# KyanChen/RSPrompter

Measured on NVIDIA H100. Metric: images/sec, higher is better.
Workload: dtype bf16

## Files before the change

rsprompter_b200/csrc/attention.cu:

```cuda
#include <cstdlib>

#include "attention.h"
#include "sm90.cuh"

namespace rsp {

constexpr float LOG2E = 1.4426950408889634f;

__device__ __forceinline__ float fast_exp2(float x) {
  float y;
  asm("ex2.approx.ftz.f32 %0, %1;" : "=f"(y) : "f"(x));
  return y;
}
__device__ __forceinline__ uint32_t pack_f16x2(float lo, float hi) {
  __half2 v = __floats2half2_rn(lo, hi);
  return *reinterpret_cast<uint32_t*>(&v);
}
__device__ __forceinline__ uint32_t bf16x2_to_f16x2(uint32_t w) {
  return pack_f16x2(__uint_as_float(w << 16), __uint_as_float(w & 0xffff0000u));
}

template <int HD, int S>
struct AttCfg {
  static constexpr int T = S * S;
  static constexpr int BM = 128;
  static constexpr int BN = 64;
  static constexpr int NQT = (T + BM - 1) / BM;
  static constexpr int NKT = (T + BN - 1) / BN;
  static constexpr int NREL = 2 * S - 1;
  static constexpr int NTAB = NREL <= 32 ? 32 : (NREL <= 64 ? 64 : 128);
  static constexpr int TAIL = HD - 64;
  static constexpr int STAGES = 4;
  static constexpr int SP = S + 4;
  __host__ __device__ static constexpr int tile_bytes(int rows) { return rows * (128 + 2 * TAIL); }
  static constexpr int STAGE_BYTES = 2 * tile_bytes(BN);
  static constexpr int smem_bytes(int qbuf) {
    return qbuf * tile_bytes(BM) + STAGES * STAGE_BYTES + 2 * tile_bytes(NTAB) + 2 * BM * SP * 4 + 8 * 64 + 1024;
  }
  static constexpr int QBUF = smem_bytes(2) <= 227 * 1024 ? 2 : 1;
  static constexpr int Q_OFF = 0;
  static constexpr int KV_OFF = Q_OFF + QBUF * tile_bytes(BM);
  static constexpr int TAB_OFF = KV_OFF + STAGES * STAGE_BYTES;
  static constexpr int BIAS_OFF = TAB_OFF + 2 * tile_bytes(NTAB);
  static constexpr int BAR_OFF = BIAS_OFF + 2 * BM * SP * 4;
  static constexpr int SMEM_BYTES = smem_bytes(QBUF);
  static constexpr int REG_PRODUCER = 40, REG_CONSUMER = 232;
  static_assert(HD == 64 || HD == 80, "head dim");
  static_assert(NREL <= 128, "table rows");
  static_assert(SMEM_BYTES <= 227 * 1024, "shared memory");
};

struct AttDev {
  __nv_bfloat16* out;
  const int* out_row_map;
  int H;
  int D;
  int n_items;
  float scale2;
};

template <int N, int TAIL>
__device__ __forceinline__ void qk_wgmma(float (&acc)[N / 2], uint32_t qa, uint32_t qtail, uint32_t b, int b_rows) {
  acc_fence(acc);
  wgmma_fence();
#pragma unroll
  for (int k = 0; k < 4; ++k)
    Wgmma<N>::template ss<0>(acc, make_gdesc(qa + 32 * k, 16, 1024), make_gdesc(b + 32 * k, 16, 1024), k);
  if constexpr (TAIL > 0)
    Wgmma<N>::template ss<0>(acc, make_gdesc_sw32(qtail, 16, 256), make_gdesc_sw32(b + b_rows * 128, 16, 256), 1);
  wgmma_commit();
  wgmma_wait<0>();
  acc_fence(acc);
}

template <int TAIL>
__device__ __forceinline__ void load_tile(uint32_t dst, int rows, const CUtensorMap* m, const CUtensorMap* mt,
                                          uint32_t bar, int col, int row, int seq) {
  tma_load_3d(dst, m, bar, col, row, seq);
  if constexpr (TAIL > 0) tma_load_3d(dst + rows * 128, mt, bar, col + 64, row, seq);
}

template <int HD, int S>
__global__ void __launch_bounds__(384, 1)
vit_attention_kernel(const __grid_constant__ CUtensorMap tm_q, const __grid_constant__ CUtensorMap tm_q_t,
                     const __grid_constant__ CUtensorMap tm_kv, const __grid_constant__ CUtensorMap tm_kv_t,
                     const __grid_constant__ CUtensorMap tm_rh, const __grid_constant__ CUtensorMap tm_rh_t,
                     const __grid_constant__ CUtensorMap tm_rw, const __grid_constant__ CUtensorMap tm_rw_t,
                     const AttDev p) {
  using C = AttCfg<HD, S>;
  constexpr int T = C::T, BM = C::BM, BN = C::BN, NKT = C::NKT, SP = C::SP, STAGES = C::STAGES, TAIL = C::TAIL;
  constexpr int QBUF = C::QBUF;
  constexpr uint32_t TILE_KV = C::tile_bytes(BN), TILE_TAB = C::tile_bytes(C::NTAB);
  extern __shared__ __align__(1024) uint8_t smem_raw[];
  uint8_t* smem = smem_raw + ((1024u - (smem_u32(smem_raw) & 1023u)) & 1023u);
  const uint32_t sbase = smem_u32(smem);
  float* relh = reinterpret_cast<float*>(smem + C::BIAS_OFF);
  float* relw = relh + BM * SP;
  uint64_t* bar_tab = reinterpret_cast<uint64_t*>(smem + C::BAR_OFF);
  uint64_t* bar_q = bar_tab + 1;
  uint64_t* bar_qe = bar_q + QBUF;
  uint64_t* bar_k = bar_qe + QBUF;
  uint64_t* bar_v = bar_k + STAGES;
  uint64_t* bar_vc = bar_v + STAGES;
  uint64_t* bar_e = bar_vc + STAGES;

  const int warp = threadIdx.x >> 5, lane = threadIdx.x & 31;
  auto decode = [&](int item, int& q0, int& head, int& seq) {
    q0 = (item % C::NQT) * BM;
    item /= C::NQT;
    head = item % p.H;
    seq = item / p.H;
  };

  if (threadIdx.x == 0) {
    tma_prefetch_desc(&tm_q);
    tma_prefetch_desc(&tm_kv);
    mbar_init(smem_u32(bar_tab), 1);
    for (int b = 0; b < QBUF; ++b) {
      mbar_init(smem_u32(&bar_q[b]), 1);
      mbar_init(smem_u32(&bar_qe[b]), 8);
    }
    for (int s = 0; s < STAGES; ++s) {
      mbar_init(smem_u32(&bar_k[s]), 1);
      mbar_init(smem_u32(&bar_v[s]), 1);
      mbar_init(smem_u32(&bar_vc[s]), 3);
      mbar_init(smem_u32(&bar_e[s]), 8);
    }
    fence_barrier_init();
  }
  __syncthreads();

  if (warp < 4) {
    setmaxnreg_dec<C::REG_PRODUCER>();
    if (warp == 0) {
      if (lane == 0) {
        const uint32_t bq = smem_u32(bar_tab);
        mbar_expect_tx(bq, 2 * TILE_TAB);
        tma_load_2d(sbase + C::TAB_OFF, &tm_rh, bq, 0, 0);
        tma_load_2d(sbase + C::TAB_OFF + TILE_TAB, &tm_rw, bq, 0, 0);
        if constexpr (TAIL > 0) {
          tma_load_2d(sbase + C::TAB_OFF + C::NTAB * 128, &tm_rh_t, bq, 64, 0);
          tma_load_2d(sbase + C::TAB_OFF + TILE_TAB + C::NTAB * 128, &tm_rw_t, bq, 64, 0);
        }
        int g = 0;
#pragma unroll 1
        for (int item = blockIdx.x, it = 0; item < p.n_items; item += gridDim.x, ++it) {
          int q0, head, seq;
          decode(item, q0, head, seq);
          const int colq = head * HD, colk = p.D + colq, colv = 2 * p.D + colq;
          const int qb = it % QBUF;
          mbar_wait(smem_u32(&bar_qe[qb]), ((it / QBUF) & 1) ^ 1);
          mbar_expect_tx(smem_u32(&bar_q[qb]), C::tile_bytes(BM));
          load_tile<TAIL>(sbase + C::Q_OFF + qb * C::tile_bytes(BM), BM, &tm_q, &tm_q_t, smem_u32(&bar_q[qb]),
                          colq, q0, seq);
#pragma unroll 1
          for (int j = 0; j < NKT; ++j, ++g) {
            const int s = g % STAGES;
            mbar_wait(smem_u32(&bar_e[s]), ((g / STAGES) & 1) ^ 1);
            const uint32_t kb = sbase + C::KV_OFF + s * C::STAGE_BYTES;
            mbar_expect_tx(smem_u32(&bar_k[s]), TILE_KV);
            load_tile<TAIL>(kb, BN, &tm_kv, &tm_kv_t, smem_u32(&bar_k[s]), colk, j * BN, seq);
            mbar_expect_tx(smem_u32(&bar_v[s]), TILE_KV);
            load_tile<TAIL>(kb + TILE_KV, BN, &tm_kv, &tm_kv_t, smem_u32(&bar_v[s]), colv, j * BN, seq);
          }
        }
      }
    } else {
      const int t = threadIdx.x - 32;
      const int n_tiles = ((p.n_items - static_cast<int>(blockIdx.x) + gridDim.x - 1) / gridDim.x) * NKT;
#pragma unroll 1
      for (int g = 0; g < n_tiles; ++g) {
        const int s = g % STAGES;
        mbar_wait(smem_u32(&bar_v[s]), (g / STAGES) & 1);
        uint4* v = reinterpret_cast<uint4*>(smem + C::KV_OFF + s * C::STAGE_BYTES + TILE_KV);
#pragma unroll 2
        for (int i = t; i < static_cast<int>(TILE_KV / 16); i += 96) {
          uint4 w = v[i];
          w.x = bf16x2_to_f16x2(w.x);
          w.y = bf16x2_to_f16x2(w.y);
          w.z = bf16x2_to_f16x2(w.z);
          w.w = bf16x2_to_f16x2(w.w);
          v[i] = w;
        }
        fence_proxy_async_smem();
        __syncwarp();
        if (lane == 0) mbar_arrive(smem_u32(&bar_vc[s]));
      }
    }
    return;
  }

  setmaxnreg_inc<C::REG_CONSUMER>();
  const int wg = (warp >> 2) - 1;
  const int r0 = wg * 64 + (warp & 3) * 16 + (lane >> 2);
  const int cq = 2 * (lane & 3);
  constexpr bool REG_W = BN % S == 0;
  constexpr int CPS = REG_W ? S / 8 : 1;
  mbar_wait(smem_u32(bar_tab), 0);
  int g = 0;
#pragma unroll 1
  for (int item = blockIdx.x, it = 0; item < p.n_items; item += gridDim.x, ++it) {
    int q0, head, seq;
    decode(item, q0, head, seq);
    const int qb = it % QBUF;
    const uint32_t qbase = sbase + C::Q_OFF + qb * C::tile_bytes(BM);
    const uint32_t qa = qbase + wg * 64 * 128;
    const uint32_t qtail = qbase + BM * 128 + wg * 64 * 32;

    mbar_wait(smem_u32(&bar_q[qb]), (it / QBUF) & 1);
    named_bar_sync(1 + wg, 128);
#pragma unroll 1
    for (int tab = 0; tab < 2; ++tab) {
      float acc[C::NTAB / 2];
      qk_wgmma<C::NTAB, TAIL>(acc, qa, qtail, sbase + C::TAB_OFF + tab * TILE_TAB, C::NTAB);
      float* dst = tab ? relw : relh;
#pragma unroll
      for (int x = 0; x < C::NTAB / 2; ++x) {
        const int r = r0 + 8 * ((x >> 1) & 1);
        const int tq = q0 + r;
        const int qc = tab ? tq % S : tq / S;
        const int t = 8 * (x >> 2) + cq + (x & 1);
        const int k = qc + S - 1 - t;
        if (t < C::NREL && k >= 0 && k < S) dst[r * SP + k] = acc[x] * LOG2E;
      }
    }
    named_bar_sync(1 + wg, 128);

    float rw[2][2 * CPS];
    if constexpr (REG_W) {
#pragma unroll
      for (int i = 0; i < 2; ++i)
#pragma unroll
        for (int m = 0; m < 2 * CPS; ++m) rw[i][m] = relw[(r0 + 8 * i) * SP + 8 * (m >> 1) + cq + (m & 1)];
    }

    float om[32], ot[8];
#pragma unroll
    for (int y = 0; y < 32; ++y) om[y] = 0.f;
#pragma unroll
    for (int y = 0; y < 8; ++y) ot[y] = 0.f;
    float m_run[2] = {-INFINITY, -INFINITY}, l_run[2] = {0.f, 0.f};
    const float scale2 = p.scale2;

#pragma unroll(REG_W ? 1 : NKT)
    for (int j = 0; j < NKT; ++j, ++g) {
      const int s = g % STAGES;
      const uint32_t ph = (g / STAGES) & 1;
      const uint32_t kb = sbase + C::KV_OFF + s * C::STAGE_BYTES, vb = kb + TILE_KV;
      mbar_wait(smem_u32(&bar_k[s]), ph);
      float sc[BN / 2];
      qk_wgmma<BN, TAIL>(sc, qa, qtail, kb, BN);
      if (j == NKT - 1) {
        __syncwarp();
        if (lane == 0) mbar_arrive(smem_u32(&bar_qe[qb]));
      }

      float mx[2] = {-INFINITY, -INFINITY};
      if constexpr (REG_W) {
        constexpr int NB = BN / S;
        float bh[2][NB];
#pragma unroll
        for (int i = 0; i < 2; ++i)
#pragma unroll
          for (int b = 0; b < NB; ++b) bh[i][b] = relh[(r0 + 8 * i) * SP + j * NB + b];
#pragma unroll
        for (int x = 0; x < BN / 2; ++x) {
          const int i = (x >> 1) & 1;
          const float t = fmaf(sc[x], scale2, bh[i][(x >> 2) / CPS] + rw[i][((x >> 2) % CPS) * 2 + (x & 1)]);
          sc[x] = t;
          mx[i] = fmaxf(mx[i], t);
        }
      } else {
#pragma unroll
        for (int x = 0; x < BN / 2; ++x) {
          const int i = (x >> 1) & 1;
          const int key = j * BN + 8 * (x >> 2) + cq + (x & 1);
          float t = -INFINITY;
          if (T % BN == 0 || key < T) {
            const int kh = key / S, kw = key - kh * S;
            const int r = r0 + 8 * i;
            t = fmaf(sc[x], scale2, relh[r * SP + kh] + relw[r * SP + kw]);
          }
          sc[x] = t;
          mx[i] = fmaxf(mx[i], t);
        }
      }
      float alpha[2];
#pragma unroll
      for (int i = 0; i < 2; ++i) {
        mx[i] = fmaxf(mx[i], __shfl_xor_sync(0xffffffffu, mx[i], 1));
        mx[i] = fmaxf(mx[i], __shfl_xor_sync(0xffffffffu, mx[i], 2));
        const float m_new = fmaxf(m_run[i], mx[i]);
        alpha[i] = fast_exp2(m_run[i] - m_new);
        m_run[i] = m_new;
        l_run[i] *= alpha[i];
      }
#pragma unroll
      for (int y = 0; y < 32; ++y) om[y] *= alpha[(y >> 1) & 1];
#pragma unroll
      for (int y = 0; y < 8; ++y) ot[y] *= alpha[(y >> 1) & 1];
      uint32_t pa[BN / 16][4];
#pragma unroll
      for (int kk = 0; kk < BN / 16; ++kk) {
#pragma unroll
        for (int h = 0; h < 4; ++h) {
          const int x = 8 * kk + 2 * h, i = h & 1;
          const float p0 = fast_exp2(sc[x] - m_run[i]), p1 = fast_exp2(sc[x + 1] - m_run[i]);
          l_run[i] += p0 + p1;
          pa[kk][h] = pack_f16x2(p0, p1);
        }
      }
      mbar_wait(smem_u32(&bar_vc[s]), ph);
      acc_fence(om);
      acc_fence(ot);
      wgmma_fence();
#pragma unroll
      for (int kk = 0; kk < BN / 16; ++kk) {
        WgmmaRsF16<64>::rs(om, pa[kk], make_gdesc(vb + kk * 2048, BN * 128, 1024));
        if constexpr (TAIL > 0) WgmmaRsF16<16>::rs(ot, pa[kk], make_gdesc_sw32(vb + BN * 128 + kk * 512, 256, 256));
      }
      wgmma_commit();
      wgmma_wait<0>();
      acc_fence(om);
      acc_fence(ot);
      __syncwarp();
      if (lane == 0) mbar_arrive(smem_u32(&bar_e[s]));
    }

#pragma unroll
    for (int i = 0; i < 2; ++i) {
      float l = l_run[i];
      l += __shfl_xor_sync(0xffffffffu, l, 1);
      l += __shfl_xor_sync(0xffffffffu, l, 2);
      const float inv = 1.0f / l;
      const int tq = q0 + r0 + 8 * i;
      if (tq >= T) continue;
      int dst = seq * T + tq;
      if (p.out_row_map) dst = __ldg(p.out_row_map + dst);
      if (dst < 0) continue;
      __nv_bfloat16* orow = p.out + static_cast<size_t>(dst) * p.D + head * HD + cq;
#pragma unroll
      for (int nb = 0; nb < 8; ++nb)
        *reinterpret_cast<uint32_t*>(orow + nb * 8) = pack_bf16x2(om[4 * nb + 2 * i] * inv, om[4 * nb + 2 * i + 1] * inv);
      if constexpr (TAIL > 0) {
#pragma unroll
        for (int nb = 0; nb < 2; ++nb)
          *reinterpret_cast<uint32_t*>(orow + 64 + nb * 8) =
              pack_bf16x2(ot[4 * nb + 2 * i] * inv, ot[4 * nb + 2 * i + 1] * inv);
      }
    }
  }
}

template <int HD, int S>
static int launch_att(const AttentionArgs& a, cudaStream_t stream) {
  using C = AttCfg<HD, S>;
  RSP_CHECK_ARG((reinterpret_cast<uintptr_t>(a.qkv) & 15) == 0 && (reinterpret_cast<uintptr_t>(a.rel_h) & 15) == 0 &&
                (reinterpret_cast<uintptr_t>(a.rel_w) & 15) == 0 && (reinterpret_cast<uintptr_t>(a.out) & 3) == 0,
                "attention: qkv / tables must be 16-byte aligned");
  AttDev p;
  p.out = static_cast<__nv_bfloat16*>(a.out);
  p.out_row_map = a.out_row_map;
  p.H = a.H; p.D = a.H * HD;
  p.scale2 = (1.0f / sqrtf(static_cast<float>(HD))) * LOG2E;
  const uint64_t ld = 3ull * p.D;
  const uint64_t qdims[3] = {ld, static_cast<uint64_t>(C::T), static_cast<uint64_t>(a.n_seq)};
  const uint64_t qstr[2] = {ld * 2, ld * 2 * C::T};
  const uint64_t tdims[2] = {static_cast<uint64_t>(HD), static_cast<uint64_t>(C::NREL)};
  const uint64_t tstr[1] = {static_cast<uint64_t>(HD) * 2};
  const uint32_t qbox[3] = {64, C::BM, 1}, qbox_t[3] = {16, C::BM, 1};
  const uint32_t kvbox[3] = {64, C::BN, 1}, kvbox_t[3] = {16, C::BN, 1};
  const uint32_t tbox[2] = {64, static_cast<uint32_t>(C::NTAB)}, tbox_t[2] = {16, static_cast<uint32_t>(C::NTAB)};
  CUtensorMap tq, tkv, th, tw, tq_t, tkv_t, th_t, tw_t;
  RSP_TRY(make_tmap_swizzled(&tq, a.qkv, 3, qdims, qstr, qbox, 0, 128));
  RSP_TRY(make_tmap_swizzled(&tkv, a.qkv, 3, qdims, qstr, kvbox, 0, 128));
  RSP_TRY(make_tmap_swizzled(&th, a.rel_h, 2, tdims, tstr, tbox, 0, 128));
  RSP_TRY(make_tmap_swizzled(&tw, a.rel_w, 2, tdims, tstr, tbox, 0, 128));
  if (C::TAIL > 0) {
    RSP_TRY(make_tmap_swizzled(&tq_t, a.qkv, 3, qdims, qstr, qbox_t, 0, 32));
    RSP_TRY(make_tmap_swizzled(&tkv_t, a.qkv, 3, qdims, qstr, kvbox_t, 0, 32));
    RSP_TRY(make_tmap_swizzled(&th_t, a.rel_h, 2, tdims, tstr, tbox_t, 0, 32));
    RSP_TRY(make_tmap_swizzled(&tw_t, a.rel_w, 2, tdims, tstr, tbox_t, 0, 32));
  } else {
    tq_t = tq; tkv_t = tkv; th_t = th; tw_t = tw;
  }
  auto kern = vit_attention_kernel<HD, S>;
  static bool attr_set_dev[kMaxDevices] = {};
  bool& attr_set = attr_set_dev[current_device()];
  if (!attr_set) {
    RSP_CHECK_CUDA(cudaFuncSetAttribute(kern, cudaFuncAttributeMaxDynamicSharedMemorySize, C::SMEM_BYTES));
    attr_set = true;
  }
  const long long items = static_cast<long long>(a.n_seq) * a.H * C::NQT;
  RSP_CHECK_ARG(items > 0 && items < (1ll << 31), "attention: %lld query tiles", items);
  p.n_items = static_cast<int>(items);
  const int grid = static_cast<int>(items < num_sms() ? items : num_sms());
  kern<<<grid, 384, C::SMEM_BYTES, stream>>>(tq, tq_t, tkv, tkv_t, th, th_t, tw, tw_t, p);
  RSP_CHECK_LAUNCH();
  return RSP_OK;
}

int vit_attention(const AttentionArgs& a, cudaStream_t stream) {
  RSP_CHECK_ARG(a.qkv && a.rel_h && a.rel_w && a.out, "attention: null pointer");
  RSP_CHECK_ARG(a.T == a.S * a.S, "attention: T=%d is not S^2 (S=%d)", a.T, a.S);
  RSP_CHECK_ARG(a.n_seq > 0 && a.H > 0, "attention: bad n_seq/H");
  if (a.S != 14 && a.S != 32 && a.S != 64)
    return vit_attention_simt(a, stream);
  if (a.hd == 64) {
    if (a.S == 64) return launch_att<64, 64>(a, stream);
    if (a.S == 32) return launch_att<64, 32>(a, stream);
    return launch_att<64, 14>(a, stream);
  }
  if (a.hd == 80) {
    if (a.S == 64) return launch_att<80, 64>(a, stream);
    if (a.S == 32) return launch_att<80, 32>(a, stream);
    return launch_att<80, 14>(a, stream);
  }
  set_last_error("attention: head dim %d unsupported (64, 80)", a.hd);
  return RSP_ERR_UNSUPPORTED;
}

__global__ void vit_attention_simt_kernel(const __nv_bfloat16* __restrict__ qkv,
                                          const __nv_bfloat16* __restrict__ rel_h,
                                          const __nv_bfloat16* __restrict__ rel_w,
                                          __nv_bfloat16* __restrict__ out, int T, int S, int H,
                                          int hd, float scale, const int* __restrict__ out_row_map) {
  const int D = H * hd;
  const int tq = blockIdx.x * blockDim.x + threadIdx.x;
  const int head = blockIdx.y;
  const int seq = blockIdx.z;
  if (tq >= T) return;
  const int qh = tq / S, qw = tq % S;
  const __nv_bfloat16* qp = qkv + (static_cast<size_t>(seq) * T + tq) * 3 * D + head * hd;
  float q[128];
  for (int d = 0; d < hd; ++d) q[d] = __bfloat162float(qp[d]);
  float rh[128], rw[128];
  for (int k = 0; k < S; ++k) {
    float ah = 0.f, aw = 0.f;
    const __nv_bfloat16* th = rel_h + static_cast<size_t>(qh - k + S - 1) * hd;
    const __nv_bfloat16* tw = rel_w + static_cast<size_t>(qw - k + S - 1) * hd;
    for (int d = 0; d < hd; ++d) {
      ah += q[d] * __bfloat162float(th[d]);
      aw += q[d] * __bfloat162float(tw[d]);
    }
    rh[k] = ah; rw[k] = aw;
  }
  float m = -INFINITY, l = 0.f;
  float o[128];
  for (int d = 0; d < hd; ++d) o[d] = 0.f;
  for (int k = 0; k < T; ++k) {
    const __nv_bfloat16* kp = qkv + (static_cast<size_t>(seq) * T + k) * 3 * D + D + head * hd;
    const __nv_bfloat16* vp = kp + D;
    float s = 0.f;
    for (int d = 0; d < hd; ++d) s += q[d] * __bfloat162float(kp[d]);
    s = s * scale + rh[k / S] + rw[k % S];
    const float mn = fmaxf(m, s);
    const float a = expf(m - mn), pe = expf(s - mn);
    l = l * a + pe;
    for (int d = 0; d < hd; ++d) o[d] = o[d] * a + pe * __bfloat162float(vp[d]);
    m = mn;
  }
  int dst = seq * T + tq;
  if (out_row_map) dst = out_row_map[dst];
  if (dst < 0) return;
  __nv_bfloat16* op = out + static_cast<size_t>(dst) * D + head * hd;
  for (int d = 0; d < hd; ++d) op[d] = __float2bfloat16_rn(o[d] / l);
}

int vit_attention_simt(const AttentionArgs& a, cudaStream_t stream) {
  RSP_CHECK_ARG(a.qkv && a.rel_h && a.rel_w && a.out, "attention_simt: null pointer");
  RSP_CHECK_ARG(a.T == a.S * a.S && a.S <= 128 && a.hd <= 128, "attention_simt: bad T/S/hd");
  dim3 block(64);
  dim3 grid((a.T + 63) / 64, a.H, a.n_seq);
  vit_attention_simt_kernel<<<grid, block, 0, stream>>>(
      static_cast<const __nv_bfloat16*>(a.qkv), static_cast<const __nv_bfloat16*>(a.rel_h),
      static_cast<const __nv_bfloat16*>(a.rel_w), static_cast<__nv_bfloat16*>(a.out), a.T, a.S, a.H,
      a.hd, 1.0f / sqrtf(static_cast<float>(a.hd)), a.out_row_map);
  RSP_CHECK_LAUNCH();
  return RSP_OK;
}
// ... 3 lines not shown
```

rsprompter_b200/csrc/sm90.cuh:

```cuda
#pragma once
#include <cuda.h>
#include <cuda_bf16.h>
#include <cuda_runtime.h>
#include <stdint.h>

namespace rsp {

__device__ __forceinline__ uint32_t smem_u32(const void* p) {
  return static_cast<uint32_t>(__cvta_generic_to_shared(p));
}

__device__ __forceinline__ uint32_t elect_one() {
  uint32_t pred = 0;
  asm volatile(
      "{\n"
      ".reg .b32 rx;\n"
      ".reg .pred px;\n"
      "elect.sync rx|px, 0xffffffff;\n"
      "selp.u32 %0, 1, 0, px;\n"
      "}\n"
      : "=r"(pred));
  return pred;
}

// ... 22 lines not shown
      "selp.u32 %0, 1, 0, p;\n"
      "}\n"
      : "=r"(ok)
      : "r"(bar), "r"(parity)
      : "memory");
  return ok;
}
__device__ __forceinline__ void mbar_wait(uint32_t bar, uint32_t parity) {
  if (mbar_try_wait(bar, parity)) return;
  long long t0 = clock64();
  uint32_t spins = 0;
  while (!mbar_try_wait(bar, parity)) {
    if ((++spins & 0x3ff) == 0 && clock64() - t0 > (1ll << 31)) __trap();
  }
}

__device__ __forceinline__ void tma_prefetch_desc(const CUtensorMap* m) {
  asm volatile("prefetch.tensormap [%0];" ::"l"(m) : "memory");
}
__device__ __forceinline__ void tma_load_2d(uint32_t dst, const CUtensorMap* m, uint32_t bar,
                                            int c0, int c1) {
  asm volatile(
      "cp.async.bulk.tensor.2d.shared::cluster.global.mbarrier::complete_tx::bytes"
      " [%0], [%1, {%3, %4}], [%2];" ::"r"(dst),
      "l"(m), "r"(bar), "r"(c0), "r"(c1)
      : "memory");
}
__device__ __forceinline__ void tma_load_3d(uint32_t dst, const CUtensorMap* m, uint32_t bar,
                                            int c0, int c1, int c2) {
  asm volatile(
      "cp.async.bulk.tensor.3d.shared::cluster.global.mbarrier::complete_tx::bytes"
      " [%0], [%1, {%3, %4, %5}], [%2];" ::"r"(dst),
      "l"(m), "r"(bar), "r"(c0), "r"(c1), "r"(c2)
      : "memory");
}
__device__ __forceinline__ void tma_load_4d(uint32_t dst, const CUtensorMap* m, uint32_t bar,
                                            int c0, int c1, int c2, int c3) {
  asm volatile(
      "cp.async.bulk.tensor.4d.shared::cluster.global.mbarrier::complete_tx::bytes"
      " [%0], [%1, {%3, %4, %5, %6}], [%2];" ::"r"(dst),
      "l"(m), "r"(bar), "r"(c0), "r"(c1), "r"(c2), "r"(c3)
      : "memory");
}

__device__ __forceinline__ void tma_store_2d(const CUtensorMap* m, uint32_t src, int c0, int c1) {
  asm volatile("cp.async.bulk.tensor.2d.global.shared::cta.bulk_group [%0, {%2, %3}], [%1];" ::"l"(m), "r"(src),
               "r"(c0), "r"(c1)
               : "memory");
}
__device__ __forceinline__ void bulk_commit() { asm volatile("cp.async.bulk.commit_group;" ::: "memory"); }
__device__ __forceinline__ void bulk_wait_read0() { asm volatile("cp.async.bulk.wait_group.read 0;" ::: "memory"); }
__device__ __forceinline__ void bulk_wait0() { asm volatile("cp.async.bulk.wait_group 0;" ::: "memory"); }

__device__ __forceinline__ uint64_t make_gdesc(uint32_t saddr, uint32_t lbo_bytes, uint32_t sbo_bytes) {
  uint64_t d = 0;
  d |= static_cast<uint64_t>((saddr & 0x3ffff) >> 4);
  d |= static_cast<uint64_t>((lbo_bytes >> 4) & 0x3fff) << 16;
  d |= static_cast<uint64_t>((sbo_bytes >> 4) & 0x3fff) << 32;
  d |= 1ull << 62;
  return d;
}

__device__ __forceinline__ uint64_t make_gdesc_sw32(uint32_t saddr, uint32_t lbo_bytes, uint32_t sbo_bytes) {
  uint64_t d = 0;
  d |= static_cast<uint64_t>((saddr & 0x3ffff) >> 4);
  d |= static_cast<uint64_t>((lbo_bytes >> 4) & 0x3fff) << 16;
  d |= static_cast<uint64_t>((sbo_bytes >> 4) & 0x3fff) << 32;
  d |= 3ull << 62;
  return d;
}

__device__ __forceinline__ void wgmma_fence() { asm volatile("wgmma.fence.sync.aligned;" ::: "memory"); }
__device__ __forceinline__ void wgmma_commit() { asm volatile("wgmma.commit_group.sync.aligned;" ::: "memory"); }
template <int N>
__device__ __forceinline__ void wgmma_wait() { asm volatile("wgmma.wait_group.sync.aligned %0;" ::"n"(N) : "memory"); }
template <int R>
__device__ __forceinline__ void acc_fence(float (&d)[R]) {
#pragma unroll
  for (int i = 0; i < R; ++i) asm volatile("" : "+f"(d[i])::"memory");
}

template <int N>
struct Wgmma;
template <> struct Wgmma<32> {
  template <int TB>
  __device__ __forceinline__ static void ss(float (&d)[16], uint64_t a, uint64_t b, uint32_t acc) {
    asm volatile(
        "{\n.reg .pred p;\n"
        "setp.ne.b32 p, %18, 0;\n"
        "wgmma.mma_async.sync.aligned.m64n32k16.f32.bf16.bf16 "
        "{" 
        "%0, %1, %2, %3, %4, %5, %6, %7, %8, %9, %10, %11, %12, %13, %14, %15"
        "}, %16, %17, p, 1, 1, 0, %19;\n}\n"
        : "+f"(d[0]), "+f"(d[1]), "+f"(d[2]), "+f"(d[3]), "+f"(d[4]), "+f"(d[5]), "+f"(d[6]), "+f"(d[7]),
          "+f"(d[8]), "+f"(d[9]), "+f"(d[10]), "+f"(d[11]), "+f"(d[12]), "+f"(d[13]), "+f"(d[14]), "+f"(d[15])
        : "l"(a), "l"(b), "r"(acc), "n"(TB));
  }
};
template <> struct Wgmma<64> {
  template <int TB>
  __device__ __forceinline__ static void ss(float (&d)[32], uint64_t a, uint64_t b, uint32_t acc) {
    asm volatile(
        "{\n.reg .pred p;\n"
        "setp.ne.b32 p, %34, 0;\n"
        "wgmma.mma_async.sync.aligned.m64n64k16.f32.bf16.bf16 "
        "{" 
        "%0, %1, %2, %3, %4, %5, %6, %7, %8, %9, %10, %11, %12, %13, %14, %15, "
        "%16, %17, %18, %19, %20, %21, %22, %23, %24, %25, %26, %27, %28, %29, %30, %31"
        "}, %32, %33, p, 1, 1, 0, %35;\n}\n"
        : "+f"(d[0]), "+f"(d[1]), "+f"(d[2]), "+f"(d[3]), "+f"(d[4]), "+f"(d[5]), "+f"(d[6]), "+f"(d[7]),
          "+f"(d[8]), "+f"(d[9]), "+f"(d[10]), "+f"(d[11]), "+f"(d[12]), "+f"(d[13]), "+f"(d[14]), "+f"(d[15]),
          "+f"(d[16]), "+f"(d[17]), "+f"(d[18]), "+f"(d[19]), "+f"(d[20]), "+f"(d[21]), "+f"(d[22]), "+f"(d[23]),
          "+f"(d[24]), "+f"(d[25]), "+f"(d[26]), "+f"(d[27]), "+f"(d[28]), "+f"(d[29]), "+f"(d[30]), "+f"(d[31])
        : "l"(a), "l"(b), "r"(acc), "n"(TB));
  }
};
template <> struct Wgmma<128> {
  template <int TB>
  __device__ __forceinline__ static void ss(float (&d)[64], uint64_t a, uint64_t b, uint32_t acc) {
    asm volatile(
        "{\n.reg .pred p;\n"
        "setp.ne.b32 p, %66, 0;\n"
        "wgmma.mma_async.sync.aligned.m64n128k16.f32.bf16.bf16 "
        "{" 
        "%0, %1, %2, %3, %4, %5, %6, %7, %8, %9, %10, %11, %12, %13, %14, %15, "
        "%16, %17, %18, %19, %20, %21, %22, %23, %24, %25, %26, %27, %28, %29, %30, %31, "
        "%32, %33, %34, %35, %36, %37, %38, %39, %40, %41, %42, %43, %44, %45, %46, %47, "
        "%48, %49, %50, %51, %52, %53, %54, %55, %56, %57, %58, %59, %60, %61, %62, %63"
        "}, %64, %65, p, 1, 1, 0, %67;\n}\n"
        : "+f"(d[0]), "+f"(d[1]), "+f"(d[2]), "+f"(d[3]), "+f"(d[4]), "+f"(d[5]), "+f"(d[6]), "+f"(d[7]),
          "+f"(d[8]), "+f"(d[9]), "+f"(d[10]), "+f"(d[11]), "+f"(d[12]), "+f"(d[13]), "+f"(d[14]), "+f"(d[15]),
          "+f"(d[16]), "+f"(d[17]), "+f"(d[18]), "+f"(d[19]), "+f"(d[20]), "+f"(d[21]), "+f"(d[22]), "+f"(d[23]),
          "+f"(d[24]), "+f"(d[25]), "+f"(d[26]), "+f"(d[27]), "+f"(d[28]), "+f"(d[29]), "+f"(d[30]), "+f"(d[31]),
          "+f"(d[32]), "+f"(d[33]), "+f"(d[34]), "+f"(d[35]), "+f"(d[36]), "+f"(d[37]), "+f"(d[38]), "+f"(d[39]),
          "+f"(d[40]), "+f"(d[41]), "+f"(d[42]), "+f"(d[43]), "+f"(d[44]), "+f"(d[45]), "+f"(d[46]), "+f"(d[47]),
          "+f"(d[48]), "+f"(d[49]), "+f"(d[50]), "+f"(d[51]), "+f"(d[52]), "+f"(d[53]), "+f"(d[54]), "+f"(d[55]),
          "+f"(d[56]), "+f"(d[57]), "+f"(d[58]), "+f"(d[59]), "+f"(d[60]), "+f"(d[61]), "+f"(d[62]), "+f"(d[63])
        : "l"(a), "l"(b), "r"(acc), "n"(TB));
  }
};
template <> struct Wgmma<256> {
  template <int TB>
  __device__ __forceinline__ static void ss(float (&d)[128], uint64_t a, uint64_t b, uint32_t acc) {
    asm volatile(
        "{\n.reg .pred p;\n"
        "setp.ne.b32 p, %130, 0;\n"
        "wgmma.mma_async.sync.aligned.m64n256k16.f32.bf16.bf16 "
        "{" 
        "%0, %1, %2, %3, %4, %5, %6, %7, %8, %9, %10, %11, %12, %13, %14, %15, "
        "%16, %17, %18, %19, %20, %21, %22, %23, %24, %25, %26, %27, %28, %29, %30, %31, "
        "%32, %33, %34, %35, %36, %37, %38, %39, %40, %41, %42, %43, %44, %45, %46, %47, "
        "%48, %49, %50, %51, %52, %53, %54, %55, %56, %57, %58, %59, %60, %61, %62, %63, "
        "%64, %65, %66, %67, %68, %69, %70, %71, %72, %73, %74, %75, %76, %77, %78, %79, "
        "%80, %81, %82, %83, %84, %85, %86, %87, %88, %89, %90, %91, %92, %93, %94, %95, "
        "%96, %97, %98, %99, %100, %101, %102, %103, %104, %105, %106, %107, %108, %109, %110, %111, "
        "%112, %113, %114, %115, %116, %117, %118, %119, %120, %121, %122, %123, %124, %125, %126, %127"
        "}, %128, %129, p, 1, 1, 0, %131;\n}\n"
        : "+f"(d[0]), "+f"(d[1]), "+f"(d[2]), "+f"(d[3]), "+f"(d[4]), "+f"(d[5]), "+f"(d[6]), "+f"(d[7]),
          "+f"(d[8]), "+f"(d[9]), "+f"(d[10]), "+f"(d[11]), "+f"(d[12]), "+f"(d[13]), "+f"(d[14]), "+f"(d[15]),
          "+f"(d[16]), "+f"(d[17]), "+f"(d[18]), "+f"(d[19]), "+f"(d[20]), "+f"(d[21]), "+f"(d[22]), "+f"(d[23]),
          "+f"(d[24]), "+f"(d[25]), "+f"(d[26]), "+f"(d[27]), "+f"(d[28]), "+f"(d[29]), "+f"(d[30]), "+f"(d[31]),
          "+f"(d[32]), "+f"(d[33]), "+f"(d[34]), "+f"(d[35]), "+f"(d[36]), "+f"(d[37]), "+f"(d[38]), "+f"(d[39]),
          "+f"(d[40]), "+f"(d[41]), "+f"(d[42]), "+f"(d[43]), "+f"(d[44]), "+f"(d[45]), "+f"(d[46]), "+f"(d[47]),
          "+f"(d[48]), "+f"(d[49]), "+f"(d[50]), "+f"(d[51]), "+f"(d[52]), "+f"(d[53]), "+f"(d[54]), "+f"(d[55]),
          "+f"(d[56]), "+f"(d[57]), "+f"(d[58]), "+f"(d[59]), "+f"(d[60]), "+f"(d[61]), "+f"(d[62]), "+f"(d[63]),
          "+f"(d[64]), "+f"(d[65]), "+f"(d[66]), "+f"(d[67]), "+f"(d[68]), "+f"(d[69]), "+f"(d[70]), "+f"(d[71]),
// ... 179 lines not shown
```

Measured before the change: 61.08.

## Add window-attention path with whole-sequence items, trimmed tail tiles, and pipelined wgmma

For the S=14 window case (T=196, not a multiple of BN), each work item now covers a whole sequence and head. All Q rows are loaded once and the K/V tiles stay resident across the query tiles. The last K/V tile is loaded with narrower TMA boxes (8 and 16 rows) and computed with a new m64n8 wgmma, so less padding is loaded and multiplied. The per-tile loop is software-pipelined so the next QK wgmma and the previous PV wgmma overlap the softmax, and relative-position biases are held in registers. In exchange it uses more shared memory for Q, more registers, and gives fewer, larger work items, which can hurt load balance.

After: 62.36, median of 6. +2.1%, better.

```diff
diff --git a/rsprompter_b200/csrc/attention.cu b/rsprompter_b200/csrc/attention.cu
--- a/rsprompter_b200/csrc/attention.cu
+++ b/rsprompter_b200/csrc/attention.cu
@@ -1,4 +1,5 @@
 #include <cstdlib>
+#include <type_traits>
 
 #include "attention.h"
 #include "sm90.cuh"
@@ -27,6 +28,10 @@
   static constexpr int BN = 64;
   static constexpr int NQT = (T + BM - 1) / BM;
   static constexpr int NKT = (T + BN - 1) / BN;
+  static constexpr bool WIN = T % BN != 0;
+  static constexpr int QROWS = WIN ? NQT * BM : BM;
+  static constexpr int KT = WIN ? (T - (NKT - 1) * BN + 7) / 8 * 8 : BN;
+  static constexpr int VT = WIN ? (T - (NKT - 1) * BN + 15) / 16 * 16 : BN;
   static constexpr int NREL = 2 * S - 1;
   static constexpr int NTAB = NREL <= 32 ? 32 : (NREL <= 64 ? 64 : 128);
   static constexpr int TAIL = HD - 64;
@@ -35,11 +40,11 @@
   __host__ __device__ static constexpr int tile_bytes(int rows) { return rows * (128 + 2 * TAIL); }
   static constexpr int STAGE_BYTES = 2 * tile_bytes(BN);
   static constexpr int smem_bytes(int qbuf) {
-    return qbuf * tile_bytes(BM) + STAGES * STAGE_BYTES + 2 * tile_bytes(NTAB) + 2 * BM * SP * 4 + 8 * 64 + 1024;
+    return qbuf * tile_bytes(QROWS) + STAGES * STAGE_BYTES + 2 * tile_bytes(NTAB) + 2 * BM * SP * 4 + 8 * 64 + 1024;
   }
   static constexpr int QBUF = smem_bytes(2) <= 227 * 1024 ? 2 : 1;
   static constexpr int Q_OFF = 0;
-  static constexpr int KV_OFF = Q_OFF + QBUF * tile_bytes(BM);
+  static constexpr int KV_OFF = Q_OFF + QBUF * tile_bytes(QROWS);
   static constexpr int TAB_OFF = KV_OFF + STAGES * STAGE_BYTES;
   static constexpr int BIAS_OFF = TAB_OFF + 2 * tile_bytes(NTAB);
   static constexpr int BAR_OFF = BIAS_OFF + 2 * BM * SP * 4;
@@ -48,6 +53,7 @@
   static_assert(HD == 64 || HD == 80, "head dim");
   static_assert(NREL <= 128, "table rows");
   static_assert(SMEM_BYTES <= 227 * 1024, "shared memory");
+  static_assert(!WIN || (S == 14 && STAGES == NKT && KT == 8 && VT == 16 && QBUF == 2), "window tiling");
 };
 
 struct AttDev {
@@ -86,11 +92,13 @@
                      const __grid_constant__ CUtensorMap tm_kv, const __grid_constant__ CUtensorMap tm_kv_t,
                      const __grid_constant__ CUtensorMap tm_rh, const __grid_constant__ CUtensorMap tm_rh_t,
                      const __grid_constant__ CUtensorMap tm_rw, const __grid_constant__ CUtensorMap tm_rw_t,
-                     const AttDev p) {
+                     const AttDev p,
+                     const __grid_constant__ CUtensorMap tm_kt, const __grid_constant__ CUtensorMap tm_kt_t,
+                     const __grid_constant__ CUtensorMap tm_vt, const __grid_constant__ CUtensorMap tm_vt_t) {
   using C = AttCfg<HD, S>;
   constexpr int T = C::T, BM = C::BM, BN = C::BN, NKT = C::NKT, SP = C::SP, STAGES = C::STAGES, TAIL = C::TAIL;
   constexpr int QBUF = C::QBUF;
-  constexpr uint32_t TILE_KV = C::tile_bytes(BN), TILE_TAB = C::tile_bytes(C::NTAB);
+  constexpr uint32_t TILE_KV = C::tile_bytes(BN), TILE_TAB = C::tile_bytes(C::NTAB), TILE_Q = C::tile_bytes(C::QROWS);
   extern __shared__ __align__(1024) uint8_t smem_raw[];
   uint8_t* smem = smem_raw + ((1024u - (smem_u32(smem_raw) & 1023u)) & 1023u);
   const uint32_t sbase = smem_u32(smem);
@@ -106,8 +114,12 @@
 
   const int warp = threadIdx.x >> 5, lane = threadIdx.x & 31;
   auto decode = [&](int item, int& q0, int& head, int& seq) {
-    q0 = (item % C::NQT) * BM;
-    item /= C::NQT;
+    if constexpr (C::WIN) {
+      q0 = 0;
+    } else {
+      q0 = (item % C::NQT) * BM;
+      item /= C::NQT;
+    }
     head = item % p.H;
     seq = item / p.H;
   };
@@ -150,18 +162,25 @@
           const int colq = head * HD, colk = p.D + colq, colv = 2 * p.D + colq;
           const int qb = it % QBUF;
           mbar_wait(smem_u32(&bar_qe[qb]), ((it / QBUF) & 1) ^ 1);
-          mbar_expect_tx(smem_u32(&bar_q[qb]), C::tile_bytes(BM));
-          load_tile<TAIL>(sbase + C::Q_OFF + qb * C::tile_bytes(BM), BM, &tm_q, &tm_q_t, smem_u32(&bar_q[qb]),
+          mbar_expect_tx(smem_u32(&bar_q[qb]), TILE_Q);
+          load_tile<TAIL>(sbase + C::Q_OFF + qb * TILE_Q, C::QROWS, &tm_q, &tm_q_t, smem_u32(&bar_q[qb]),
                           colq, q0, seq);
 #pragma unroll 1
           for (int j = 0; j < NKT; ++j, ++g) {
             const int s = g % STAGES;
             mbar_wait(smem_u32(&bar_e[s]), ((g / STAGES) & 1) ^ 1);
             const uint32_t kb = sbase + C::KV_OFF + s * C::STAGE_BYTES;
-            mbar_expect_tx(smem_u32(&bar_k[s]), TILE_KV);
-            load_tile<TAIL>(kb, BN, &tm_kv, &tm_kv_t, smem_u32(&bar_k[s]), colk, j * BN, seq);
-            mbar_expect_tx(smem_u32(&bar_v[s]), TILE_KV);
-            load_tile<TAIL>(kb + TILE_KV, BN, &tm_kv, &tm_kv_t, smem_u32(&bar_v[s]), colv, j * BN, seq);
+            if (C::WIN && j == NKT - 1) {
+              mbar_expect_tx(smem_u32(&bar_k[s]), C::tile_bytes(C::KT));
+              load_tile<TAIL>(kb, C::KT, &tm_kt, &tm_kt_t, smem_u32(&bar_k[s]), colk, j * BN, seq);
+              mbar_expect_tx(smem_u32(&bar_v[s]), C::tile_bytes(C::VT));
+              load_tile<TAIL>(kb + TILE_KV, C::VT, &tm_vt, &tm_vt_t, smem_u32(&bar_v[s]), colv, j * BN, seq);
+            } else {
+              mbar_expect_tx(smem_u32(&bar_k[s]), TILE_KV);
+              load_tile<TAIL>(kb, BN, &tm_kv, &tm_kv_t, smem_u32(&bar_k[s]), colk, j * BN, seq);
+              mbar_expect_tx(smem_u32(&bar_v[s]), TILE_KV);
+              load_tile<TAIL>(kb + TILE_KV, BN, &tm_kv, &tm_kv_t, smem_u32(&bar_v[s]), colv, j * BN, seq);
+            }
           }
         }
       }
@@ -173,8 +192,9 @@
         const int s = g % STAGES;
         mbar_wait(smem_u32(&bar_v[s]), (g / STAGES) & 1);
         uint4* v = reinterpret_cast<uint4*>(smem + C::KV_OFF + s * C::STAGE_BYTES + TILE_KV);
+        const int n16 = (C::WIN && g % NKT == NKT - 1 ? C::tile_bytes(C::VT) : TILE_KV) / 16;
 #pragma unroll 2
-        for (int i = t; i < static_cast<int>(TILE_KV / 16); i += 96) {
+        for (int i = t; i < n16; i += 96) {
           uint4 w = v[i];
           w.x = bf16x2_to_f16x2(w.x);
           w.y = bf16x2_to_f16x2(w.y);
@@ -194,20 +214,8 @@
   const int wg = (warp >> 2) - 1;
   const int r0 = wg * 64 + (warp & 3) * 16 + (lane >> 2);
   const int cq = 2 * (lane & 3);
-  constexpr bool REG_W = BN % S == 0;
-  constexpr int CPS = REG_W ? S / 8 : 1;
-  mbar_wait(smem_u32(bar_tab), 0);
-  int g = 0;
-#pragma unroll 1
-  for (int item = blockIdx.x, it = 0; item < p.n_items; item += gridDim.x, ++it) {
-    int q0, head, seq;
-    decode(item, q0, head, seq);
-    const int qb = it % QBUF;
-    const uint32_t qbase = sbase + C::Q_OFF + qb * C::tile_bytes(BM);
-    const uint32_t qa = qbase + wg * 64 * 128;
-    const uint32_t qtail = qbase + BM * 128 + wg * 64 * 32;
-
-    mbar_wait(smem_u32(&bar_q[qb]), (it / QBUF) & 1);
+
+  auto gather_bias = [&](uint32_t qa, uint32_t qtail, int q0) {
     named_bar_sync(1 + wg, 128);
 #pragma unroll 1
     for (int tab = 0; tab < 2; ++tab) {
@@ -225,108 +233,27 @@
       }
     }
     named_bar_sync(1 + wg, 128);
-
-    float rw[2][2 * CPS];
-    if constexpr (REG_W) {
-#pragma unroll
-      for (int i = 0; i < 2; ++i)
-#pragma unroll
-        for (int m = 0; m < 2 * CPS; ++m) rw[i][m] = relw[(r0 + 8 * i) * SP + 8 * (m >> 1) + cq + (m & 1)];
-    }
-
-    float om[32], ot[8];
-#pragma unroll
-    for (int y = 0; y < 32; ++y) om[y] = 0.f;
-#pragma unroll
-    for (int y = 0; y < 8; ++y) ot[y] = 0.f;
-    float m_run[2] = {-INFINITY, -INFINITY}, l_run[2] = {0.f, 0.f};
-    const float scale2 = p.scale2;
-
-#pragma unroll(REG_W ? 1 : NKT)
-    for (int j = 0; j < NKT; ++j, ++g) {
-      const int s = g % STAGES;
-      const uint32_t ph = (g / STAGES) & 1;
-      const uint32_t kb = sbase + C::KV_OFF + s * C::STAGE_BYTES, vb = kb + TILE_KV;
-      mbar_wait(smem_u32(&bar_k[s]), ph);
-      float sc[BN / 2];
-      qk_wgmma<BN, TAIL>(sc, qa, qtail, kb, BN);
-      if (j == NKT - 1) {
-        __syncwarp();
-        if (lane == 0) mbar_arrive(smem_u32(&bar_qe[qb]));
-      }
-
-      float mx[2] = {-INFINITY, -INFINITY};
-      if constexpr (REG_W) {
-        constexpr int NB = BN / S;
-        float bh[2][NB];
-#pragma unroll
-        for (int i = 0; i < 2; ++i)
-#pragma unroll
-          for (int b = 0; b < NB; ++b) bh[i][b] = relh[(r0 + 8 * i) * SP + j * NB + b];
-#pragma unroll
-        for (int x = 0; x < BN / 2; ++x) {
-          const int i = (x >> 1) & 1;
-          const float t = fmaf(sc[x], scale2, bh[i][(x >> 2) / CPS] + rw[i][((x >> 2) % CPS) * 2 + (x & 1)]);
-          sc[x] = t;
-          mx[i] = fmaxf(mx[i], t);
-        }
-      } else {
-#pragma unroll
-        for (int x = 0; x < BN / 2; ++x) {
-          const int i = (x >> 1) & 1;
-          const int key = j * BN + 8 * (x >> 2) + cq + (x & 1);
-          float t = -INFINITY;
-          if (T % BN == 0 || key < T) {
-            const int kh = key / S, kw = key - kh * S;
-            const int r = r0 + 8 * i;
-            t = fmaf(sc[x], scale2, relh[r * SP + kh] + relw[r * SP + kw]);
-          }
-          sc[x] = t;
-          mx[i] = fmaxf(mx[i], t);
-        }
-      }
-      float alpha[2];
-#pragma unroll
-      for (int i = 0; i < 2; ++i) {
-        mx[i] = fmaxf(mx[i], __shfl_xor_sync(0xffffffffu, mx[i], 1));
-        mx[i] = fmaxf(mx[i], __shfl_xor_sync(0xffffffffu, mx[i], 2));
-        const float m_new = fmaxf(m_run[i], mx[i]);
-        alpha[i] = fast_exp2(m_run[i] - m_new);
-        m_run[i] = m_new;
-        l_run[i] *= alpha[i];
-      }
-#pragma unroll
-      for (int y = 0; y < 32; ++y) om[y] *= alpha[(y >> 1) & 1];
-#pragma unroll
-      for (int y = 0; y < 8; ++y) ot[y] *= alpha[(y >> 1) & 1];
-      uint32_t pa[BN / 16][4];
-#pragma unroll
-      for (int kk = 0; kk < BN / 16; ++kk) {
-#pragma unroll
-        for (int h = 0; h < 4; ++h) {
-          const int x = 8 * kk + 2 * h, i = h & 1;
-          const float p0 = fast_exp2(sc[x] - m_run[i]), p1 = fast_exp2(sc[x + 1] - m_run[i]);
-          l_run[i] += p0 + p1;
-          pa[kk][h] = pack_f16x2(p0, p1);
-        }
-      }
-      mbar_wait(smem_u32(&bar_vc[s]), ph);
-      acc_fence(om);
-      acc_fence(ot);
-      wgmma_fence();
-#pragma unroll
-      for (int kk = 0; kk < BN / 16; ++kk) {
-        WgmmaRsF16<64>::rs(om, pa[kk], make_gdesc(vb + kk * 2048, BN * 128, 1024));
-        if constexpr (TAIL > 0) WgmmaRsF16<16>::rs(ot, pa[kk], make_gdesc_sw32(vb + BN * 128 + kk * 512, 256, 256));
-      }
-      wgmma_commit();
-      wgmma_wait<0>();
-      acc_fence(om);
-      acc_fence(ot);
-      __syncwarp();
-      if (lane == 0) mbar_arrive(smem_u32(&bar_e[s]));
-    }
-
+  };
+
+  auto rescale = [&](float (&mx)[2], float (&m_run)[2], float (&l_run)[2], float (&om)[32], float (&ot)[8]) {
+    float alpha[2];
+#pragma unroll
+    for (int i = 0; i < 2; ++i) {
+      mx[i] = fmaxf(mx[i], __shfl_xor_sync(0xffffffffu, mx[i], 1));
+      mx[i] = fmaxf(mx[i], __shfl_xor_sync(0xffffffffu, mx[i], 2));
+      const float m_new = fmaxf(m_run[i], mx[i]);
+      alpha[i] = fast_exp2(m_run[i] - m_new);
+      m_run[i] = m_new;
+      l_run[i] *= alpha[i];
+    }
+#pragma unroll
+    for (int y = 0; y < 32; ++y) om[y] *= alpha[(y >> 1) & 1];
+#pragma unroll
+    for (int y = 0; y < 8; ++y) ot[y] *= alpha[(y >> 1) & 1];
+  };
+
+  auto store_out = [&](const float (&om)[32], const float (&ot)[8], const float (&l_run)[2], int q0, int head,
+                       int seq) {
 #pragma unroll
     for (int i = 0; i < 2; ++i) {
       float l = l_run[i];
@@ -348,6 +275,280 @@
           *reinterpret_cast<uint32_t*>(orow + 64 + nb * 8) =
               pack_bf16x2(ot[4 * nb + 2 * i] * inv, ot[4 * nb + 2 * i + 1] * inv);
       }
+    }
+  };
+
+  mbar_wait(smem_u32(bar_tab), 0);
+  int g = 0;
+
+  if constexpr (C::WIN) {
+#pragma unroll 1
+    for (int item = blockIdx.x, it = 0; item < p.n_items; item += gridDim.x, ++it, g += NKT) {
+      int q00, head, seq;
+      decode(item, q00, head, seq);
+      const int qb = it % QBUF;
+      const uint32_t qbase = sbase + C::Q_OFF + qb * TILE_Q;
+      const uint32_t ph = (g / STAGES) & 1;
+      mbar_wait(smem_u32(&bar_q[qb]), (it / QBUF) & 1);
+#pragma unroll 1
+      for (int qt = 0; qt < C::NQT; ++qt) {
+        const bool last_qt = qt == C::NQT - 1;
+        const int q0 = qt * BM, qrow = q0 + wg * 64;
+        gather_bias(qbase + qrow * 128, qbase + C::QROWS * 128 + qrow * 32, q0);
+        float rh[2][S], rw[2][S];
+#pragma unroll
+        for (int i = 0; i < 2; ++i) {
+#pragma unroll
+          for (int a = 0; a < S; ++a) {
+            const int kw = a + cq;
+            rh[i][a] = relh[(r0 + 8 * i) * SP + a];
+            rw[i][a] = relw[(r0 + 8 * i) * SP + (kw < S ? kw : kw - S)];
+          }
+        }
+
+        float om[32], ot[8];
+#pragma unroll
+        for (int y = 0; y < 32; ++y) om[y] = 0.f;
+#pragma unroll
+        for (int y = 0; y < 8; ++y) ot[y] = 0.f;
+        float m_run[2] = {-INFINITY, -INFINITY}, l_run[2] = {0.f, 0.f};
+        const float scale2 = p.scale2;
+
+        const uint32_t qa = qbase + qrow * 128, qtail = qbase + C::QROWS * 128 + qrow * 32;
+
+        auto issue_qk = [&](auto jc, auto& sc) {
+          constexpr int j = decltype(jc)::value;
+          constexpr int NK = j < NKT - 1 ? BN : C::KT;
+          const uint32_t kb = sbase + C::KV_OFF + j * C::STAGE_BYTES;
+          mbar_wait(smem_u32(&bar_k[j]), ph);
+          acc_fence(sc);
+          wgmma_fence();
+#pragma unroll
+          for (int k = 0; k < 4; ++k)
+            Wgmma<NK>::template ss<0>(sc, make_gdesc(qa + 32 * k, 16, 1024), make_gdesc(kb + 32 * k, 16, 1024), k);
+          if constexpr (TAIL > 0)
+            Wgmma<NK>::template ss<0>(sc, make_gdesc_sw32(qtail, 16, 256), make_gdesc_sw32(kb + NK * 128, 16, 256), 1);
+          wgmma_commit();
+        };
+
+        auto softmax = [&](auto jc, auto& sc, auto& pa, float (&alpha)[2]) {
+          constexpr int j = decltype(jc)::value;
+          constexpr int NK = j < NKT - 1 ? BN : C::KT;
+          float mx[2] = {-INFINITY, -INFINITY};
+#pragma unroll
+          for (int x = 0; x < NK / 2; ++x) {
+            const int i = (x >> 1) & 1;
+            const int c = j * BN + 8 * (x >> 2) + (x & 1), a = c / S, b = c % S;
+            const float h = (b + 6 >= S && b + cq >= S) ? rh[i][a + 1 < S ? a + 1 : S - 1] : rh[i][a];
+            float t = fmaf(sc[x], scale2, h + rw[i][b]);
+            if (j == NKT - 1 && c + cq >= T) t = -INFINITY;
+            sc[x] = t;
+            mx[i] = fmaxf(mx[i], t);
+          }
+#pragma unroll
+          for (int i = 0; i < 2; ++i) {
+            mx[i] = fmaxf(mx[i], __shfl_xor_sync(0xffffffffu, mx[i], 1));
+            mx[i] = fmaxf(mx[i], __shfl_xor_sync(0xffffffffu, mx[i], 2));
+            const float m_new = fmaxf(m_run[i], mx[i]);
+            alpha[i] = fast_exp2(m_run[i] - m_new);
+            m_run[i] = m_new;
+            l_run[i] *= alpha[i];
+          }
+#pragma unroll
+          for (int kk = 0; kk < (NK + 15) / 16; ++kk) {
+#pragma unroll
+            for (int h = 0; h < 4; ++h) {
+              const int x = 8 * kk + 2 * h, i = h & 1;
+              if (x < NK / 2) {
+                const float p0 = fast_exp2(sc[x] - m_run[i]), p1 = fast_exp2(sc[x + 1] - m_run[i]);
+                l_run[i] += p0 + p1;
+                pa[kk][h] = pack_f16x2(p0, p1);
+              } else {
+                pa[kk][h] = 0u;
+              }
+            }
+          }
+        };
+
+        auto issue_pv = [&](auto jc, auto& pa, const float (&alpha)[2]) {
+          constexpr int j = decltype(jc)::value;
+          constexpr int NV = j < NKT - 1 ? BN : C::VT;
+          const uint32_t vb = sbase + C::KV_OFF + j * C::STAGE_BYTES + TILE_KV;
+#pragma unroll
+          for (int y = 0; y < 32; ++y) om[y] *= alpha[(y >> 1) & 1];
+#pragma unroll
+          for (int y = 0; y < 8; ++y) ot[y] *= alpha[(y >> 1) & 1];
+          mbar_wait(smem_u32(&bar_vc[j]), ph);
+          acc_fence(om);
+          acc_fence(ot);
+#pragma unroll
+          for (int kk = 0; kk < (NV + 15) / 16; ++kk)
+#pragma unroll
+            for (int h = 0; h < 4; ++h) asm volatile("" : "+r"(pa[kk][h]));
+          wgmma_fence();
+#pragma unroll
+          for (int kk = 0; kk < (NV + 15) / 16; ++kk) {
+            WgmmaRsF16<64>::rs(om, pa[kk], make_gdesc(vb + kk * 2048, NV * 128, 1024));
+            if constexpr (TAIL > 0) WgmmaRsF16<16>::rs(ot, pa[kk], make_gdesc_sw32(vb + NV * 128 + kk * 512, 256, 256));
+          }
+          wgmma_commit();
+        };
+
+        auto retire_pv = [&](int j, auto& pa) {
+          acc_fence(om);
+          acc_fence(ot);
+#pragma unroll
+          for (int kk = 0; kk < static_cast<int>(sizeof(pa) / sizeof(pa[0])); ++kk)
+#pragma unroll
+            for (int h = 0; h < 4; ++h) asm volatile("" : "+r"(pa[kk][h]));
+          if (last_qt) {
+            __syncwarp();
+            if (lane == 0) mbar_arrive(smem_u32(&bar_e[j]));
+          }
+        };
+
+        using I0 = std::integral_constant<int, 0>;
+        using I1 = std::integral_constant<int, 1>;
+        using I2 = std::integral_constant<int, 2>;
+        using I3 = std::integral_constant<int, 3>;
+        static_assert(NKT == 4, "window key tiles");
+        float s0[BN / 2], s1[BN / 2], s2[BN / 2], s3[C::KT / 2], alpha[2];
+        uint32_t p0[BN / 16][4], p1[BN / 16][4], p2[BN / 16][4], p3[1][4];
+        issue_qk(I0(), s0);
+        wgmma_wait<0>();
+        acc_fence(s0);
+        issue_qk(I1(), s1);
+        softmax(I0(), s0, p0, alpha);
+        issue_pv(I0(), p0, alpha);
+        wgmma_wait<1>();
+        acc_fence(s1);
+        issue_qk(I2(), s2);
+        softmax(I1(), s1, p1, alpha);
+        wgmma_wait<1>();
+        retire_pv(0, p0);
+        issue_pv(I1(), p1, alpha);
+        wgmma_wait<1>();
+        acc_fence(s2);
+        issue_qk(I3(), s3);
+        softmax(I2(), s2, p2, alpha);
+        wgmma_wait<1>();
+        retire_pv(1, p1);
+        issue_pv(I2(), p2, alpha);
+        wgmma_wait<1>();
+        acc_fence(s3);
+        if (last_qt) {
+          __syncwarp();
+          if (lane == 0) mbar_arrive(smem_u32(&bar_qe[qb]));
+        }
+        softmax(I3(), s3, p3, alpha);
+        wgmma_wait<0>();
+        retire_pv(2, p2);
+        issue_pv(I3(), p3, alpha);
+        wgmma_wait<0>();
+        retire_pv(3, p3);
+        store_out(om, ot, l_run, q0, head, seq);
+      }
+    }
+  } else {
+    constexpr int CPS = S / 8;
+#pragma unroll 1
+    for (int item = blockIdx.x, it = 0; item < p.n_items; item += gridDim.x, ++it) {
+      int q0, head, seq;
+      decode(item, q0, head, seq);
+      const int qb = it % QBUF;
+      const uint32_t qbase = sbase + C::Q_OFF + qb * TILE_Q;
+      const uint32_t qa = qbase + wg * 64 * 128;
+      const uint32_t qtail = qbase + BM * 128 + wg * 64 * 32;
+
+      mbar_wait(smem_u32(&bar_q[qb]), (it / QBUF) & 1);
+      named_bar_sync(1 + wg, 128);
+#pragma unroll 1
+      for (int tab = 0; tab < 2; ++tab) {
+        float acc[C::NTAB / 2];
+        qk_wgmma<C::NTAB, TAIL>(acc, qa, qtail, sbase + C::TAB_OFF + tab * TILE_TAB, C::NTAB);
+        float* dst = tab ? relw : relh;
+#pragma unroll
+        for (int x = 0; x < C::NTAB / 2; ++x) {
+          const int r = r0 + 8 * ((x >> 1) & 1);
+          const int tq = q0 + r;
+          const int qc = tab ? tq % S : tq / S;
+          const int t = 8 * (x >> 2) + cq + (x & 1);
+          const int k = qc + S - 1 - t;
+          if (t < C::NREL && k >= 0 && k < S) dst[r * SP + k] = acc[x] * LOG2E;
+        }
+      }
+      named_bar_sync(1 + wg, 128);
+
+      float rw[2][2 * CPS];
+#pragma unroll
+      for (int i = 0; i < 2; ++i)
+#pragma unroll
+        for (int m = 0; m < 2 * CPS; ++m) rw[i][m] = relw[(r0 + 8 * i) * SP + 8 * (m >> 1) + cq + (m & 1)];
+
+      float om[32], ot[8];
+#pragma unroll
+      for (int y = 0; y < 32; ++y) om[y] = 0.f;
+#pragma unroll
+      for (int y = 0; y < 8; ++y) ot[y] = 0.f;
+      float m_run[2] = {-INFINITY, -INFINITY}, l_run[2] = {0.f, 0.f};
+      const float scale2 = p.scale2;
+
+#pragma unroll 1
+      for (int j = 0; j < NKT; ++j, ++g) {
+        const int s = g % STAGES;
+        const uint32_t ph = (g / STAGES) & 1;
+        const uint32_t kb = sbase + C::KV_OFF + s * C::STAGE_BYTES, vb = kb + TILE_KV;
+        mbar_wait(smem_u32(&bar_k[s]), ph);
+        float sc[BN / 2];
+        qk_wgmma<BN, TAIL>(sc, qa, qtail, kb, BN);
+        if (j == NKT - 1) {
+          __syncwarp();
+          if (lane == 0) mbar_arrive(smem_u32(&bar_qe[qb]));
+        }
+
+        float mx[2] = {-INFINITY, -INFINITY};
+        constexpr int NB = BN / S;
+        float bh[2][NB];
+#pragma unroll
+        for (int i = 0; i < 2; ++i)
+#pragma unroll
+          for (int b = 0; b < NB; ++b) bh[i][b] = relh[(r0 + 8 * i) * SP + j * NB + b];
+#pragma unroll
+        for (int x = 0; x < BN / 2; ++x) {
+          const int i = (x >> 1) & 1;
+          const float t = fmaf(sc[x], scale2, bh[i][(x >> 2) / CPS] + rw[i][((x >> 2) % CPS) * 2 + (x & 1)]);
+          sc[x] = t;
+          mx[i] = fmaxf(mx[i], t);
+        }
+        rescale(mx, m_run, l_run, om, ot);
+        uint32_t pa[BN / 16][4];
+#pragma unroll
+        for (int kk = 0; kk < BN / 16; ++kk) {
+#pragma unroll
+          for (int h = 0; h < 4; ++h) {
+            const int x = 8 * kk + 2 * h, i = h & 1;
+            const float p0 = fast_exp2(sc[x] - m_run[i]), p1 = fast_exp2(sc[x + 1] - m_run[i]);
+            l_run[i] += p0 + p1;
+            pa[kk][h] = pack_f16x2(p0, p1);
+          }
+        }
+        mbar_wait(smem_u32(&bar_vc[s]), ph);
+        acc_fence(om);
+        acc_fence(ot);
+        wgmma_fence();
+#pragma unroll
+        for (int kk = 0; kk < BN / 16; ++kk) {
+          WgmmaRsF16<64>::rs(om, pa[kk], make_gdesc(vb + kk * 2048, BN * 128, 1024));
+          if constexpr (TAIL > 0) WgmmaRsF16<16>::rs(ot, pa[kk], make_gdesc_sw32(vb + BN * 128 + kk * 512, 256, 256));
+        }
+        wgmma_commit();
+        wgmma_wait<0>();
+        acc_fence(om);
+        acc_fence(ot);
+        __syncwarp();
+        if (lane == 0) mbar_arrive(smem_u32(&bar_e[s]));
+      }
+      store_out(om, ot, l_run, q0, head, seq);
     }
   }
 }
@@ -368,10 +569,12 @@
   const uint64_t qstr[2] = {ld * 2, ld * 2 * C::T};
   const uint64_t tdims[2] = {static_cast<uint64_t>(HD), static_cast<uint64_t>(C::NREL)};
   const uint64_t tstr[1] = {static_cast<uint64_t>(HD) * 2};
-  const uint32_t qbox[3] = {64, C::BM, 1}, qbox_t[3] = {16, C::BM, 1};
+  const uint32_t qbox[3] = {64, C::QROWS, 1}, qbox_t[3] = {16, C::QROWS, 1};
   const uint32_t kvbox[3] = {64, C::BN, 1}, kvbox_t[3] = {16, C::BN, 1};
+  const uint32_t ktbox[3] = {64, C::KT, 1}, ktbox_t[3] = {16, C::KT, 1};
+  const uint32_t vtbox[3] = {64, C::VT, 1}, vtbox_t[3] = {16, C::VT, 1};
   const uint32_t tbox[2] = {64, static_cast<uint32_t>(C::NTAB)}, tbox_t[2] = {16, static_cast<uint32_t>(C::NTAB)};
-  CUtensorMap tq, tkv, th, tw, tq_t, tkv_t, th_t, tw_t;
+  CUtensorMap tq, tkv, th, tw, tq_t, tkv_t, th_t, tw_t, tkt, tkt_t, tvt, tvt_t;
   RSP_TRY(make_tmap_swizzled(&tq, a.qkv, 3, qdims, qstr, qbox, 0, 128));
   RSP_TRY(make_tmap_swizzled(&tkv, a.qkv, 3, qdims, qstr, kvbox, 0, 128));
   RSP_TRY(make_tmap_swizzled(&th, a.rel_h, 2, tdims, tstr, tbox, 0, 128));
@@ -384,6 +587,18 @@
   } else {
     tq_t = tq; tkv_t = tkv; th_t = th; tw_t = tw;
   }
+  if (C::WIN) {
+    RSP_TRY(make_tmap_swizzled(&tkt, a.qkv, 3, qdims, qstr, ktbox, 0, 128));
+    RSP_TRY(make_tmap_swizzled(&tvt, a.qkv, 3, qdims, qstr, vtbox, 0, 128));
+    if (C::TAIL > 0) {
+      RSP_TRY(make_tmap_swizzled(&tkt_t, a.qkv, 3, qdims, qstr, ktbox_t, 0, 32));
+      RSP_TRY(make_tmap_swizzled(&tvt_t, a.qkv, 3, qdims, qstr, vtbox_t, 0, 32));
+    } else {
+      tkt_t = tkt; tvt_t = tvt;
+    }
+  } else {
+    tkt = tkt_t = tvt = tvt_t = tkv;
+  }
   auto kern = vit_attention_kernel<HD, S>;
   static bool attr_set_dev[kMaxDevices] = {};
   bool& attr_set = attr_set_dev[current_device()];
@@ -391,11 +606,11 @@
     RSP_CHECK_CUDA(cudaFuncSetAttribute(kern, cudaFuncAttributeMaxDynamicSharedMemorySize, C::SMEM_BYTES));
     attr_set = true;
   }
-  const long long items = static_cast<long long>(a.n_seq) * a.H * C::NQT;
-  RSP_CHECK_ARG(items > 0 && items < (1ll << 31), "attention: %lld query tiles", items);
+  const long long items = static_cast<long long>(a.n_seq) * a.H * (C::WIN ? 1 : C::NQT);
+  RSP_CHECK_ARG(items > 0 && items < (1ll << 31), "attention: %lld work items", items);
   p.n_items = static_cast<int>(items);
   const int grid = static_cast<int>(items < num_sms() ? items : num_sms());
-  kern<<<grid, 384, C::SMEM_BYTES, stream>>>(tq, tq_t, tkv, tkv_t, th, th_t, tw, tw_t, p);
+  kern<<<grid, 384, C::SMEM_BYTES, stream>>>(tq, tq_t, tkv, tkv_t, th, th_t, tw, tw_t, p, tkt, tkt_t, tvt, tvt_t);
   RSP_CHECK_LAUNCH();
   return RSP_OK;
 }
diff --git a/rsprompter_b200/csrc/sm90.cuh b/rsprompter_b200/csrc/sm90.cuh
--- a/rsprompter_b200/csrc/sm90.cuh
+++ b/rsprompter_b200/csrc/sm90.cuh
@@ -128,6 +128,18 @@
 
 template <int N>
 struct Wgmma;
+template <> struct Wgmma<8> {
+  template <int TB>
+  __device__ __forceinline__ static void ss(float (&d)[4], uint64_t a, uint64_t b, uint32_t acc) {
+    asm volatile(
+        "{\n.reg .pred p;\n"
+        "setp.ne.b32 p, %6, 0;\n"
+        "wgmma.mma_async.sync.aligned.m64n8k16.f32.bf16.bf16 "
+        "{%0, %1, %2, %3}, %4, %5, p, 1, 1, 0, %7;\n}\n"
+        : "+f"(d[0]), "+f"(d[1]), "+f"(d[2]), "+f"(d[3])
+        : "l"(a), "l"(b), "r"(acc), "n"(TB));
+  }
+};
 template <> struct Wgmma<32> {
   template <int TB>
   __device__ __forceinline__ static void ss(float (&d)[16], uint64_t a, uint64_t b, uint32_t acc) {
```
